# eikehmueller/IncompressibleEulerHDG

Hardware: AMD Instinct MI355X
Metric: million DOF-updates/sec (HDG-IMEX k=2, 1024^2 tri mesh) (higher is better)
Workload: dtype f64

## Files before the change

### incompressibleeulerhdg_amd/csrc/hdg_trace_tile.hpp

```cpp
#pragma once
#include <hip/hip_runtime.h>

namespace hdg {

template <int K>
struct TraceTile {
  static constexpr int NL = Dim<K>::NL, NT = 3 * NL;
  static constexpr int TW = 16, TH = 8, NTHREADS = 256;
  static constexpr int W2 = TW + 4, H2 = TH + 4, N2 = W2 * H2;
  static constexpr int WPE_POST = K == 1 ? 5 : (K == 2 ? 4 : (K == 3 ? 3 : 1));
  static constexpr int W3 = TW + 6, H3 = TH + 6, N3 = W3 * H3;
  static constexpr int W1 = TW + 2, H1 = TH + 2, N1 = W1 * H1;
  static constexpr int KMAX = (N2 + NTHREADS - 1) / NTHREADS;
};

template <int K, int RW, int RH>
__device__ __forceinline__ void lds_trace_stencil(const double* __restrict__ A, int li, int lj, bool in_x, bool in_y, bool below,
                                                  bool left, const DevTables& T, double* own, double* yH, double* yV, double* yD) {
  constexpr int NL = Dim<K>::NL, NT = 3 * NL;
  auto at = [&](int t, int m, int dj, int di) { return A[((t * NL + m) * RH + (lj + dj)) * RW + (li + di)]; };
  double uA[NT], uB[NT], uC[NT];
#pragma unroll
  for (int m = 0; m < NL; m++) {
    own[m] = at(0, m, 0, 0); own[NL + m] = at(2, m, 0, 0); own[2 * NL + m] = at(1, m, 0, 0);
    uA[m] = at(0, m, 1, 0); uA[2 * NL + m] = at(1, m, 0, 1);
    uB[NL + m] = at(2, m, -1, 0); uB[2 * NL + m] = at(1, m, -1, 1);
    uC[m] = at(0, m, 1, -1); uC[NL + m] = at(2, m, 0, -1);
    yH[m] = yV[m] = yD[m] = 0.0;
  }
  const bool vL = in_x && in_y, vB = in_x && below, vW = in_y && left;
#pragma unroll
  for (int m = 0; m < NL; m++) {
    if (!in_x) own[m] = 0.0;
    if (!vL) own[NL + m] = 0.0;
    if (!in_y) own[2 * NL + m] = 0.0;
    uA[NL + m] = own[NL + m];
    uB[m] = own[m];
    uC[2 * NL + m] = own[2 * NL + m];
  }
  const double* __restrict__ SL = T.SK[0];
  const double* __restrict__ SU = T.SK[1];
  if (vL) {
    mv_acc_ld<NL, NT>(SL + 0 * NL * NT, NT, own, yH, -1.0);
    mv_acc_ld<NL, NT>(SL + 1 * NL * NT, NT, own, yD, -1.0);
    mv_acc_ld<NL, NT>(SL + 2 * NL * NT, NT, own, yV, -1.0);
    mv_acc_ld<NL, NT>(SU + 1 * NL * NT, NT, uA, yD, -1.0);
  }
  if (vB) mv_acc_ld<NL, NT>(SU + 0 * NL * NT, NT, uB, yH, -1.0);
  if (vW) mv_acc_ld<NL, NT>(SU + 2 * NL * NT, NT, uC, yV, -1.0);
}

#define HDG_TILE_OF_BLOCK                                              \
  const int tiles_per_xcd_ = (int)(gridDim.x >> 3);                    \
  const int tile_v = (int)(blockIdx.x & 7) * tiles_per_xcd_ + (int)(blockIdx.x >> 3); \
  if (tile_v >= ntx * nty) return;                                     \
  const int tile_y = tile_v / ntx, tile_x = tile_v - tile_y * ntx;
struct CornerInfo {
  bool exists, in_x, in_y, below, left;
  bool own_x;
  int vH, vV;
  long o;
};
struct TileRows {
  int jlo, jhi, rlo, rhi;
};
__device__ __forceinline__ CornerInfo corner_info(const Geo& g, const TileRows& tr, int i, int j) {
  CornerInfo c;
  const int gj = g.joff + j;
  if (g.px) {
    c.exists = gj >= 0 && gj <= g.nyg && j >= tr.rlo && j < tr.rhi;
    c.own_x = i >= 0 && i < g.nx;
    const int iw = i < 0 ? i + g.nx : (i >= g.nx ? i - g.nx : i);
    c.in_x = c.exists;
    c.in_y = c.exists && gj < g.nyg;
    c.below = gj > 0;
    c.left = true;
    c.vH = gj == 0 ? 1 : (gj == g.nyg ? 2 : 0);
    c.vV = 0;
    c.o = (long)(j + GH) * g.P + iw;
    return c;
  }
  c.exists = i >= 0 && i <= g.nx && gj >= 0 && gj <= g.nyg && j >= tr.rlo && j < tr.rhi;
  c.own_x = true;
  c.in_x = c.exists && i < g.nx;
  c.in_y = c.exists && gj < g.nyg;
  c.below = gj > 0;
  c.left = i > 0;
  c.vH = gj == 0 ? 1 : (gj == g.nyg ? 2 : 0);
  c.vV = i == 0 ? 1 : (i == g.nx ? 2 : 0);
  c.o = (long)(j + GH) * g.P + i;
  return c;
}
template <int NL>
__device__ __forceinline__ void load_corner(const double* __restrict__ v, const Geo& g, const CornerInfo& c, double* e) {
#pragma unroll
  for (int m = 0; m < NL; m++) {
    e[m] = c.in_x ? v[((long)0 * NL + m) * g.G + c.o] : 0.0;
    e[NL + m] = (c.in_x && c.in_y) ? v[((long)2 * NL + m) * g.G + c.o] : 0.0;
    e[2 * NL + m] = c.in_y ? v[((long)1 * NL + m) * g.G + c.o] : 0.0;
  }
}
template <int NL>
__device__ __forceinline__ void store_corner(double* __restrict__ v, const Geo& g, const CornerInfo& c, const double* e) {
#pragma unroll
  for (int m = 0; m < NL; m++) {
    v[((long)0 * NL + m) * g.G + c.o] = c.in_x ? e[m] : 0.0;
    v[((long)2 * NL + m) * g.G + c.o] = (c.in_x && c.in_y) ? e[NL + m] : 0.0;
    v[((long)1 * NL + m) * g.G + c.o] = c.in_y ? e[2 * NL + m] : 0.0;
  }
}
template <int NL>
__device__ __forceinline__ void corner_dinv(const DevTables& T, const CornerInfo& c, double sc, const double* r, double* z) {
#pragma unroll
  for (int q = 0; q < 3 * NL; q++) z[q] = 0.0;
  mv_acc_ld<NL, NL>(T.trDinv[0][0], NL, r, z, sc);
  mv_acc_ld<NL, NL>(T.trDinv[2][0], NL, r + NL, z + NL, sc);
  mv_acc_ld<NL, NL>(T.trDinv[1][0], NL, r + 2 * NL, z + 2 * NL, sc);
  if (c.vH != 0) {
#pragma unroll
    for (int q = 0; q < NL; q++) z[q] = 0.0;
    mv_acc_ld<NL, NL>(T.trDinv[0][c.vH], NL, r, z, sc);
  }
  if (c.vV != 0) {
#pragma unroll
    for (int q = 0; q < NL; q++) z[2 * NL + q] = 0.0;
    mv_acc_ld<NL, NL>(T.trDinv[1][c.vV], NL, r + 2 * NL, z + 2 * NL, sc);
  }
}
template <int NL>
__device__ __forceinline__ int plane_of(int q) { return q < NL ? q : (q < 2 * NL ? 2 * NL + (q - NL) : NL + (q - 2 * NL)); }

template <int K>
__global__ __launch_bounds__(TraceTile<K>::NTHREADS) void k_trace_pre_tile(int ntx, int nty, Geo g, TileRows tr, DevTables T, const double* __restrict__ r, double c0, double c1,
                                                         double c2, double* __restrict__ z_out, double* __restrict__ res_out) {
  typedef TraceTile<K> TT;
  constexpr int NL = TT::NL, NT = TT::NT, TW = TT::TW, TH = TT::TH, W2 = TT::W2, H2 = TT::H2, W1 = TT::W1, H1 = TT::H1, KMAX = TT::KMAX;
  __shared__ double Ds[NT * TT::N2];
  __shared__ double Zs[NT * TT::N1];
  HDG_TILE_OF_BLOCK
  const int i0 = tile_x * TW, j0 = tr.jlo + tile_y * TH;
  double rr[KMAX][NT], dd[KMAX][NT];
#pragma unroll
  for (int k = 0; k < KMAX; k++) {
    const int idx = threadIdx.x + k * TT::NTHREADS;
    if (idx < TT::N2) {
      const int lj = idx / W2, li = idx - lj * W2;
      const int jc = j0 - 2 + lj;
      const CornerInfo c = corner_info(g, tr, i0 - 2 + li, jc);
      load_corner<NL>(r, g, c, rr[k]);
      corner_dinv<NL>(T, c, c0, rr[k], dd[k]);
#pragma unroll
      for (int q = 0; q < NT; q++) Ds[(plane_of<NL>(q) * H2 + lj) * W2 + li] = dd[k][q];
    }
  }
  __syncthreads();
#pragma unroll
  for (int k = 0; k < KMAX; k++) {
    const int idx = threadIdx.x + k * TT::NTHREADS;
    if (idx < TT::N2) {
      const int lj = idx / W2, li = idx - lj * W2;
      if (li >= 1 && li < W2 - 1 && lj >= 1 && lj < H2 - 1) {
        const int jc = j0 - 2 + lj;
        const CornerInfo c = corner_info(g, tr, i0 - 2 + li, jc);
        double z[NT];
#pragma unroll
        for (int q = 0; q < NT; q++) z[q] = 0.0;
        if (c.exists) {
          double own[NT], y[3][NL], r1[NT], zz[NT];
          lds_trace_stencil<K, W2, H2>(Ds, li, lj, c.in_x, c.in_y, c.below, c.left, T, own, y[0], y[1], y[2]);
#pragma unroll
          for (int m = 0; m < NL; m++) {
            r1[m] = rr[k][m] - y[0][m];
            r1[NL + m] = rr[k][NL + m] - y[2][m];
            r1[2 * NL + m] = rr[k][2 * NL + m] - y[1][m];
          }
          corner_dinv<NL>(T, c, c2, r1, zz);
#pragma unroll
          for (int q = 0; q < NT; q++) z[q] = dd[k][q] + fma(c1, dd[k][q], zz[q]);
        }
#pragma unroll
        for (int q = 0; q < NT; q++) Zs[(plane_of<NL>(q) * H1 + (lj - 1)) * W1 + (li - 1)] = z[q];
        if (c.exists && c.own_x && li >= 2 && li < W2 - 2 && lj >= 2 && lj < H2 - 2 && jc < tr.jhi) store_corner<NL>(z_out, g, c, z);
      }
    }
  }
  __syncthreads();
#pragma unroll
  for (int k = 0; k < KMAX; k++) {
    const int idx = threadIdx.x + k * TT::NTHREADS;
    if (idx < TT::N2) {
      const int lj = idx / W2, li = idx - lj * W2;
      if (li >= 2 && li < W2 - 2 && lj >= 2 && lj < H2 - 2) {
        const int jc = j0 - 2 + lj;
        const CornerInfo c = corner_info(g, tr, i0 - 2 + li, jc);
        if (c.exists && c.own_x && jc < tr.jhi) {
          double own[NT], y[3][NL], res[NT];
          lds_trace_stencil<K, W1, H1>(Zs, li - 1, lj - 1, c.in_x, c.in_y, c.below, c.left, T, own, y[0], y[1], y[2]);
#pragma unroll
          for (int m = 0; m < NL; m++) {
            res[m] = rr[k][m] - y[0][m];
            res[NL + m] = rr[k][NL + m] - y[2][m];
            res[2 * NL + m] = rr[k][2 * NL + m] - y[1][m];
          }
          store_corner<NL>(res_out, g, c, res);
        }
      }
    }
  }
}

template <int K, bool DOTS>
__global__ __launch_bounds__(TraceTile<K>::NTHREADS) __attribute__((amdgpu_waves_per_eu(TraceTile<K>::WPE_POST))) void k_trace_post_tile(int ntx, int nty, Geo g, TileRows tr, DevTables T, const double* __restrict__ z_in, const double* __restrict__ r,
                                                          const double* __restrict__ xc, double sH, double sV, double sD, double c0,
                                                          double c1, double c2, double* __restrict__ z_out, double* __restrict__ w_out,
                                                          double* __restrict__ part) {
  typedef TraceTile<K> TT;
  constexpr int NL = TT::NL, NT = TT::NT, TW = TT::TW, TH = TT::TH, W2 = TT::W2, H2 = TT::H2, W3 = TT::W3, H3 = TT::H3, KMAX = TT::KMAX;
  __shared__ double Zs[NT * TT::N3];
  __shared__ double Ds[NT * TT::N2];
  HDG_TILE_OF_BLOCK
  const int i0 = tile_x * TW, j0 = tr.jlo + tile_y * TH;
  const int st = g.nx + 1;
  for (int idx = threadIdx.x; idx < TT::N3; idx += TT::NTHREADS) {
    const int lj = idx / W3, li = idx - lj * W3;
    const int i = i0 - 3 + li, j = j0 - 3 + lj;
    const CornerInfo c = corner_info(g, tr, i, j);
    double z[NT];
    load_corner<NL>(z_in, g, c, z);
    if (c.exists && g.px) {
      const int n = g.nx, m = g.nx, jg = g.pj0 + j;
      const int iw = i < 0 ? i + n : (i >= n ? i - n : i), i1 = iw + 1 == n ? 0 : iw + 1;
      const int jw = jg < 0 ? jg + m : (jg >= m ? jg - m : jg), j1 = jw + 1 == m ? 0 : jw + 1;
      const double v00 = xc[(long)jw * n + iw], v10 = xc[(long)jw * n + i1], v01 = xc[(long)j1 * n + iw];
      edge_prolong(v00, v10, sH, z);
      if (c.in_y) edge_prolong(v10, v01, sD, z + NL);
      if (c.in_y) edge_prolong(v00, v01, sV, z + 2 * NL);
    } else if (c.exists) {
      const long J = g.joff + j;
      const double v00 = xc[J * st + i];
      const double v10 = c.in_x ? xc[J * st + i + 1] : 0.0, v01 = c.in_y ? xc[(J + 1) * st + i] : 0.0;
      if (c.in_x) edge_prolong(v00, v10, sH, z);
      if (c.in_x && c.in_y) edge_prolong(v10, v01, sD, z + NL);
      if (c.in_y) edge_prolong(v00, v01, sV, z + 2 * NL);
    }
#pragma unroll
    for (int q = 0; q < NT; q++) Zs[(plane_of<NL>(q) * H3 + lj) * W3 + li] = z[q];
  }
  double r0[KMAX][NT];
#pragma unroll
  for (int k = 0; k < KMAX; k++) {
    const int idx = threadIdx.x + k * TT::NTHREADS;
    const int lj = idx / W2, li = idx - lj * W2;
    CornerInfo c = corner_info(g, tr, i0 - 2 + li, j0 - 2 + lj);
    if (idx >= TT::N2) c.in_x = c.in_y = false;
    load_corner<NL>(r, g, c, r0[k]);
  }
  __syncthreads();
  double dots[5] = {0.0, 0.0, 0.0, 0.0, 0.0};
#pragma unroll
  for (int k = 0; k < KMAX; k++) {
    const int idx = threadIdx.x + k * TT::NTHREADS;
    if (idx < TT::N2) {
      const int lj = idx / W2, li = idx - lj * W2;
      const int jc = j0 - 2 + lj;
      const CornerInfo c = corner_info(g, tr, i0 - 2 + li, jc);
      double d0[NT];
#pragma unroll
      for (int q = 0; q < NT; q++) d0[q] = 0.0;
      if (c.exists) {
        double own[NT], y[3][NL];
        lds_trace_stencil<K, W3, H3>(Zs, li + 1, lj + 1, c.in_x, c.in_y, c.below, c.left, T, own, y[0], y[1], y[2]);
#pragma unroll
        for (int m = 0; m < NL; m++) {
          r0[k][m] -= y[0][m];
          r0[k][NL + m] -= y[2][m];
          r0[k][2 * NL + m] -= y[1][m];
        }
        corner_dinv<NL>(T, c, c0, r0[k], d0);
      }
#pragma unroll
      for (int q = 0; q < NT; q++) Ds[(plane_of<NL>(q) * H2 + lj) * W2 + li] = d0[q];
    }
  }
  __syncthreads();
#pragma unroll
  for (int k = 0; k < KMAX; k++) {
    const int idx = threadIdx.x + k * TT::NTHREADS;
    if (idx < TT::N2) {
      const int lj = idx / W2, li = idx - lj * W2;
      if (li >= 1 && li < W2 - 1 && lj >= 1 && lj < H2 - 1) {
        const int jc = j0 - 2 + lj;
        const CornerInfo c = corner_info(g, tr, i0 - 2 + li, jc);
        double z2[NT];
#pragma unroll
        for (int q = 0; q < NT; q++) z2[q] = 0.0;
        if (c.exists) {
          double own[NT], y[3][NL], r1[NT], zz[NT];
          lds_trace_stencil<K, W2, H2>(Ds, li, lj, c.in_x, c.in_y, c.below, c.left, T, own, y[0], y[1], y[2]);
#pragma unroll
          for (int m = 0; m < NL; m++) {
            r1[m] = r0[k][m] - y[0][m];
            r1[NL + m] = r0[k][NL + m] - y[2][m];
            r1[2 * NL + m] = r0[k][2 * NL + m] - y[1][m];
          }
          corner_dinv<NL>(T, c, c2, r1, zz);
#pragma unroll
          for (int q = 0; q < NT; q++) {
            const double z1 = Zs[(plane_of<NL>(q) * H3 + (lj + 1)) * W3 + (li + 1)] + own[q];
            z2[q] = z1 + fma(c1, own[q], zz[q]);
          }
        }
#pragma unroll
        for (int q = 0; q < NT; q++) Zs[(plane_of<NL>(q) * H3 + (lj + 1)) * W3 + (li + 1)] = z2[q];
        if (c.exists && c.own_x && li >= 2 && li < W2 - 2 && lj >= 2 && lj < H2 - 2 && jc < tr.jhi) store_corner<NL>(z_out, g, c, z2);
      }
    }
  }
  if (!w_out) return;
  double rr3[KMAX][NT];
  if (DOTS) {
#pragma unroll
    for (int k = 0; k < KMAX; k++) {
      const int idx = threadIdx.x + k * TT::NTHREADS;
      const int lj = idx / W2, li = idx - lj * W2;
      const int jc = j0 - 2 + lj;
      CornerInfo c = corner_info(g, tr, i0 - 2 + li, jc);
      if (!(idx < TT::N2 && li >= 2 && li < W2 - 2 && lj >= 2 && lj < H2 - 2 && c.exists && c.own_x && jc < tr.jhi)) c.in_x = c.in_y = false;
      load_corner<NL>(r, g, c, rr3[k]);
    }
  }
  __syncthreads();
#pragma unroll
  for (int k = 0; k < KMAX; k++) {
    const int idx = threadIdx.x + k * TT::NTHREADS;
    if (idx < TT::N2) {
      const int lj = idx / W2, li = idx - lj * W2;
      if (li >= 2 && li < W2 - 2 && lj >= 2 && lj < H2 - 2) {
        const int jc = j0 - 2 + lj;
        const CornerInfo c = corner_info(g, tr, i0 - 2 + li, jc);
        if (c.exists && c.own_x && jc < tr.jhi) {
          double own[NT], y[3][NL], w[NT];
          lds_trace_stencil<K, W3, H3>(Zs, li + 1, lj + 1, c.in_x, c.in_y, c.below, c.left, T, own, y[0], y[1], y[2]);
#pragma unroll
          for (int m = 0; m < NL; m++) { w[m] = y[0][m]; w[NL + m] = y[2][m]; w[2 * NL + m] = y[1][m]; }
          store_corner<NL>(w_out, g, c, w);
          if (DOTS) {
            const double* rr = rr3[k];
            dots[0] += sH * own[0] + sD * own[NL] + sV * own[2 * NL];
            dots[4] += sH * rr[0] + sD * rr[NL] + sV * rr[2 * NL];
#pragma unroll
            for (int q = 0; q < NT; q++) {
              const double zq = own[q];
              dots[1] = fma(zq, rr[q], dots[1]);
              dots[2] = fma(zq, zq, dots[2]);
              dots[3] = fma(zq, w[q], dots[3]);
            }
          }
        }
      }
    }
  }
  if (DOTS) {
    __shared__ double sm[TT::NTHREADS / 64][5];
    const int lane = threadIdx.x & 63, wv = threadIdx.x >> 6;
#pragma unroll
    for (int q = 0; q < 5; q++) {
      const double sv = wave_sum(dots[q]);
      if (lane == 0) sm[wv][q] = sv;
    }
    __syncthreads();
    if (threadIdx.x < 5) {
      double sv = 0.0;
      for (int w2 = 0; w2 < TT::NTHREADS / 64; w2++) sv += sm[w2][threadIdx.x];
      part[(long)threadIdx.x * (ntx * nty) + tile_v] = sv;
    }
  }
}

}
```

Before: 819.5.

## Remap threads to tile corners interior-first to cut divergence in halo stages

Threads are now assigned to tile corners in an interior-first, then ring-by-ring order instead of row-major. Each stage's active set (full halo, one-ring halo, interior) then becomes a contiguous prefix of thread ids. Whole wavefronts can skip the stages they take no part in, instead of being partly masked. To keep the dot-product reduction in the same order as before, per-corner partial dots are staged through shared memory and regathered in row-major order, which adds an extra barrier and some LDS traffic.

```diff
diff --git a/incompressibleeulerhdg_amd/csrc/hdg_trace_tile.hpp b/incompressibleeulerhdg_amd/csrc/hdg_trace_tile.hpp
--- a/incompressibleeulerhdg_amd/csrc/hdg_trace_tile.hpp
+++ b/incompressibleeulerhdg_amd/csrc/hdg_trace_tile.hpp
@@ -1,17 +1,48 @@
 #pragma once
+#ifdef __HIPCC__
 #include <hip/hip_runtime.h>
+#define HDG_TILE_HD __host__ __device__
+#else
+#define HDG_TILE_HD
+#endif
 
 namespace hdg {
 
-template <int K>
-struct TraceTile {
-  static constexpr int NL = Dim<K>::NL, NT = 3 * NL;
+struct TileCorner {
+  int li, lj;
+};
+struct TileShape {
   static constexpr int TW = 16, TH = 8, NTHREADS = 256;
   static constexpr int W2 = TW + 4, H2 = TH + 4, N2 = W2 * H2;
-  static constexpr int WPE_POST = K == 1 ? 5 : (K == 2 ? 4 : (K == 3 ? 3 : 1));
   static constexpr int W3 = TW + 6, H3 = TH + 6, N3 = W3 * H3;
   static constexpr int W1 = TW + 2, H1 = TH + 2, N1 = W1 * H1;
+  static constexpr int N0 = TW * TH;
   static constexpr int KMAX = (N2 + NTHREADS - 1) / NTHREADS;
+  static HDG_TILE_HD constexpr TileCorner corner(int idx) {
+    if (idx < N0) return TileCorner{2 + idx % TW, 2 + idx / TW};
+    const int h = idx < N1 ? 1 : 2;
+    const int s = idx - (h == 1 ? N0 : N1), o = 2 - h, w = TW + 2 * h, e = TH + 2 * h;
+    if (s < w) return TileCorner{o + s, o};
+    if (s < 2 * w) return TileCorner{o + s - w, o + e - 1};
+    const int t = s - 2 * w;
+    return t < e - 2 ? TileCorner{o, o + 1 + t} : TileCorner{o + w - 1, o + 1 + t - (e - 2)};
+  }
+  static HDG_TILE_HD constexpr int tile_slot(int li, int lj) {
+    return (li >= 2 && li < W2 - 2 && lj >= 2 && lj < H2 - 2) ? (lj - 2) * TW + (li - 2) : -1;
+  }
+  static HDG_TILE_HD constexpr int row_major_slot(int t) { return t < N2 ? tile_slot(t % W2, t / W2) : -1; }
+};
+
+}
+
+#ifdef __HIPCC__
+namespace hdg {
+
+template <int K>
+struct TraceTile : TileShape {
+  static constexpr int NL = Dim<K>::NL, NT = 3 * NL;
+  static constexpr int WPE_POST = K == 1 ? 5 : (K == 2 ? 4 : (K == 3 ? 3 : 1));
+  static_assert(KMAX == 1 && 5 * N0 <= NT * N2, "one corner per thread; the per-corner inner-product values fit into Ds");
 };
 
 template <int K, int RW, int RH>
@@ -130,6 +161,11 @@
 template <int NL>
 __device__ __forceinline__ int plane_of(int q) { return q < NL ? q : (q < 2 * NL ? 2 * NL + (q - NL) : NL + (q - 2 * NL)); }
 
+__device__ __forceinline__ int held_corner(int idx) {
+  const TileCorner c = TileShape::corner(idx);
+  return c.li | (c.lj << 8);
+}
+
 template <int K>
 __global__ __launch_bounds__(TraceTile<K>::NTHREADS) void k_trace_pre_tile(int ntx, int nty, Geo g, TileRows tr, DevTables T, const double* __restrict__ r, double c0, double c1,
                                                          double c2, double* __restrict__ z_out, double* __restrict__ res_out) {
@@ -139,12 +175,13 @@
   __shared__ double Zs[NT * TT::N1];
   HDG_TILE_OF_BLOCK
   const int i0 = tile_x * TW, j0 = tr.jlo + tile_y * TH;
+  const int tid = (int)threadIdx.x, me = held_corner(tid);
   double rr[KMAX][NT], dd[KMAX][NT];
 #pragma unroll
   for (int k = 0; k < KMAX; k++) {
-    const int idx = threadIdx.x + k * TT::NTHREADS;
-    if (idx < TT::N2) {
-      const int lj = idx / W2, li = idx - lj * W2;
+    const int idx = tid + k * TT::NTHREADS;
+    if (idx < TT::N2) {
+      const int li = me & 255, lj = me >> 8;
       const int jc = j0 - 2 + lj;
       const CornerInfo c = corner_info(g, tr, i0 - 2 + li, jc);
       load_corner<NL>(r, g, c, rr[k]);
@@ -156,10 +193,10 @@
   __syncthreads();
 #pragma unroll
   for (int k = 0; k < KMAX; k++) {
-    const int idx = threadIdx.x + k * TT::NTHREADS;
-    if (idx < TT::N2) {
-      const int lj = idx / W2, li = idx - lj * W2;
-      if (li >= 1 && li < W2 - 1 && lj >= 1 && lj < H2 - 1) {
+    const int idx = tid + k * TT::NTHREADS;
+    if (idx < TT::N2) {
+      const int li = me & 255, lj = me >> 8;
+      if (idx < TT::N1) {
         const int jc = j0 - 2 + lj;
         const CornerInfo c = corner_info(g, tr, i0 - 2 + li, jc);
         double z[NT];
@@ -180,17 +217,17 @@
         }
 #pragma unroll
         for (int q = 0; q < NT; q++) Zs[(plane_of<NL>(q) * H1 + (lj - 1)) * W1 + (li - 1)] = z[q];
-        if (c.exists && c.own_x && li >= 2 && li < W2 - 2 && lj >= 2 && lj < H2 - 2 && jc < tr.jhi) store_corner<NL>(z_out, g, c, z);
+        if (c.exists && c.own_x && idx < TT::N0 && jc < tr.jhi) store_corner<NL>(z_out, g, c, z);
       }
     }
   }
   __syncthreads();
 #pragma unroll
   for (int k = 0; k < KMAX; k++) {
-    const int idx = threadIdx.x + k * TT::NTHREADS;
-    if (idx < TT::N2) {
-      const int lj = idx / W2, li = idx - lj * W2;
-      if (li >= 2 && li < W2 - 2 && lj >= 2 && lj < H2 - 2) {
+    const int idx = tid + k * TT::NTHREADS;
+    if (idx < TT::N2) {
+      const int li = me & 255, lj = me >> 8;
+      if (idx < TT::N0) {
         const int jc = j0 - 2 + lj;
         const CornerInfo c = corner_info(g, tr, i0 - 2 + li, jc);
         if (c.exists && c.own_x && jc < tr.jhi) {
@@ -220,6 +257,7 @@
   __shared__ double Ds[NT * TT::N2];
   HDG_TILE_OF_BLOCK
   const int i0 = tile_x * TW, j0 = tr.jlo + tile_y * TH;
+  const int tid = (int)threadIdx.x, me = held_corner(tid);
   const int st = g.nx + 1;
   for (int idx = threadIdx.x; idx < TT::N3; idx += TT::NTHREADS) {
     const int lj = idx / W3, li = idx - lj * W3;
@@ -249,8 +287,8 @@
   double r0[KMAX][NT];
 #pragma unroll
   for (int k = 0; k < KMAX; k++) {
-    const int idx = threadIdx.x + k * TT::NTHREADS;
-    const int lj = idx / W2, li = idx - lj * W2;
+    const int idx = tid + k * TT::NTHREADS;
+    const int li = me & 255, lj = me >> 8;
     CornerInfo c = corner_info(g, tr, i0 - 2 + li, j0 - 2 + lj);
     if (idx >= TT::N2) c.in_x = c.in_y = false;
     load_corner<NL>(r, g, c, r0[k]);
@@ -259,9 +297,9 @@
   double dots[5] = {0.0, 0.0, 0.0, 0.0, 0.0};
 #pragma unroll
   for (int k = 0; k < KMAX; k++) {
-    const int idx = threadIdx.x + k * TT::NTHREADS;
-    if (idx < TT::N2) {
-      const int lj = idx / W2, li = idx - lj * W2;
+    const int idx = tid + k * TT::NTHREADS;
+    if (idx < TT::N2) {
+      const int li = me & 255, lj = me >> 8;
       const int jc = j0 - 2 + lj;
       const CornerInfo c = corner_info(g, tr, i0 - 2 + li, jc);
       double d0[NT];
@@ -285,10 +323,10 @@
   __syncthreads();
 #pragma unroll
   for (int k = 0; k < KMAX; k++) {
-    const int idx = threadIdx.x + k * TT::NTHREADS;
-    if (idx < TT::N2) {
-      const int lj = idx / W2, li = idx - lj * W2;
-      if (li >= 1 && li < W2 - 1 && lj >= 1 && lj < H2 - 1) {
+    const int idx = tid + k * TT::NTHREADS;
+    if (idx < TT::N2) {
+      const int li = me & 255, lj = me >> 8;
+      if (idx < TT::N1) {
         const int jc = j0 - 2 + lj;
         const CornerInfo c = corner_info(g, tr, i0 - 2 + li, jc);
         double z2[NT];
@@ -312,7 +350,7 @@
         }
 #pragma unroll
         for (int q = 0; q < NT; q++) Zs[(plane_of<NL>(q) * H3 + (lj + 1)) * W3 + (li + 1)] = z2[q];
-        if (c.exists && c.own_x && li >= 2 && li < W2 - 2 && lj >= 2 && lj < H2 - 2 && jc < tr.jhi) store_corner<NL>(z_out, g, c, z2);
+        if (c.exists && c.own_x && idx < TT::N0 && jc < tr.jhi) store_corner<NL>(z_out, g, c, z2);
       }
     }
   }
@@ -321,21 +359,23 @@
   if (DOTS) {
 #pragma unroll
     for (int k = 0; k < KMAX; k++) {
-      const int idx = threadIdx.x + k * TT::NTHREADS;
-      const int lj = idx / W2, li = idx - lj * W2;
-      const int jc = j0 - 2 + lj;
-      CornerInfo c = corner_info(g, tr, i0 - 2 + li, jc);
-      if (!(idx < TT::N2 && li >= 2 && li < W2 - 2 && lj >= 2 && lj < H2 - 2 && c.exists && c.own_x && jc < tr.jhi)) c.in_x = c.in_y = false;
-      load_corner<NL>(r, g, c, rr3[k]);
+      const int idx = tid + k * TT::NTHREADS;
+      if (idx < TT::N0) {
+        const int li = me & 255, lj = me >> 8;
+        const int jc = j0 - 2 + lj;
+        CornerInfo c = corner_info(g, tr, i0 - 2 + li, jc);
+        if (!(c.exists && c.own_x && jc < tr.jhi)) c.in_x = c.in_y = false;
+        load_corner<NL>(r, g, c, rr3[k]);
+      }
     }
   }
   __syncthreads();
 #pragma unroll
   for (int k = 0; k < KMAX; k++) {
-    const int idx = threadIdx.x + k * TT::NTHREADS;
-    if (idx < TT::N2) {
-      const int lj = idx / W2, li = idx - lj * W2;
-      if (li >= 2 && li < W2 - 2 && lj >= 2 && lj < H2 - 2) {
+    const int idx = tid + k * TT::NTHREADS;
+    if (idx < TT::N2) {
+      const int li = me & 255, lj = me >> 8;
+      if (idx < TT::N0) {
         const int jc = j0 - 2 + lj;
         const CornerInfo c = corner_info(g, tr, i0 - 2 + li, jc);
         if (c.exists && c.own_x && jc < tr.jhi) {
@@ -357,11 +397,19 @@
             }
           }
         }
+        if (DOTS) {
+#pragma unroll
+          for (int q = 0; q < 5; q++) Ds[q * TT::N0 + idx] = dots[q];
+        }
       }
     }
   }
   if (DOTS) {
     __shared__ double sm[TT::NTHREADS / 64][5];
+    __syncthreads();
+    const int slot = TT::row_major_slot((int)threadIdx.x);
+#pragma unroll
+    for (int q = 0; q < 5; q++) dots[q] = slot >= 0 ? Ds[q * TT::N0 + slot] : 0.0;
     const int lane = threadIdx.x & 63, wv = threadIdx.x >> 6;
 #pragma unroll
     for (int q = 0; q < 5; q++) {
@@ -378,3 +426,4 @@
 }
 
 }
+#endif
```

Result: no change. 825.8, median of 6 (+0.8%).
